# jscant/PointVS

Hardware: AMD Instinct MI355X
Metric: protein-ligand graphs/sec fwd+bwd (+Adam step), 3-layer EGNN ch=32, ~2k nodes r=10A (higher is better)
Workload: dtype f32

## Files before the change

### pointvs_amd/csrc/graph_prepare.hip

```cpp
#include "common.h"
#include "profile.h"
#include <hipcub/hipcub.hpp>

namespace {

__global__ void k_extract(const int64_t* __restrict__ ei, const int64_t* __restrict__ ea, int A,
                          int N, int E, int32_t* row32, int32_t* col32, int32_t* ids,
                          uint8_t* etype_in, int32_t* status) {
    int e = blockIdx.x * blockDim.x + threadIdx.x;
    if (e >= E) return;
    int64_t r = ei[e], c = ei[(size_t)E + e];
    int bad = 0;
    if (r < 0 || r >= N || c < 0 || c >= N) { bad |= 1; r = 0; c = 0; }
    row32[e] = (int32_t)r;
    col32[e] = (int32_t)c;
    ids[e] = e;
    if (A > 0) {
        int hot = -1, ones = 0, other = 0;
        for (int a = 0; a < A; ++a) {
            int64_t v = ea[(size_t)e * A + a];
            if (v == 1) { ones++; hot = a; }
            else if (v != 0) other = 1;
        }
        if (ones != 1 || other) { bad |= 2; if (hot < 0) hot = 0; }
// ... 208 lines not shown
    int p = blockIdx.x * blockDim.x + threadIdx.x;
    if (p < E) iota[p] = p;
}

__global__ void k_init_split(int n_graphs, const int32_t* __restrict__ edge_ptr, int32_t* __restrict__ split,
                             int32_t* __restrict__ status) {
    const int g = blockIdx.x * blockDim.x + threadIdx.x;
    if (g == 0) *status = 0;
    if (g < n_graphs) split[g] = edge_ptr[g + 1];
}

__global__ void k_run_starts(const int64_t* __restrict__ rows, int N, int E, int n_graphs,
                             const int32_t* __restrict__ status, const int32_t* __restrict__ node_ptr,
                             const int32_t* __restrict__ edge_ptr, const int32_t* __restrict__ split,
                             int2* __restrict__ rec, int32_t* __restrict__ unsafe,
                             int32_t* __restrict__ rowptr, float* __restrict__ inv_deg) {
    const int n = blockIdx.x * blockDim.x + threadIdx.x;
    if (n >= N) return;
    if (n == N - 1) rowptr[N] = E;
    const bool broken = (*status & 5) != 0;
    if (n == 0) *unsafe = broken;
    if (broken) {
        rec[n] = make_int2(0, 0);
        rowptr[n] = n == 0 ? 0 : E;
        inv_deg[n] = 1.0f;
        return;
    }
    int lo = 0, hi = n_graphs;
    while (hi - lo > 1) {
        const int mid = (lo + hi) >> 1;
        if (node_ptr[mid] <= n) lo = mid; else hi = mid;
    }
    const int g = lo;
    const int a0 = edge_ptr[g], a1 = split[g], b1 = edge_ptr[g + 1];
    int f0 = a0, l0 = a1, f1 = a0, l1 = a1, f2 = a1, l2 = b1, f3 = a1, l3 = b1;
    while (f0 < l0 || f1 < l1 || f2 < l2 || f3 < l3) {
        const int m0 = (f0 + l0) >> 1, m1 = (f1 + l1) >> 1, m2 = (f2 + l2) >> 1, m3 = (f3 + l3) >> 1;
        const int64_t v0 = f0 < l0 ? rows[m0] : 0, v1 = f1 < l1 ? rows[m1] : 0;
        const int64_t v2 = f2 < l2 ? rows[m2] : 0, v3 = f3 < l3 ? rows[m3] : 0;
        if (f0 < l0) { if (v0 < n) f0 = m0 + 1; else l0 = m0; }
        if (f1 < l1) { if (v1 < n + 1) f1 = m1 + 1; else l1 = m1; }
        if (f2 < l2) { if (v2 < n) f2 = m2 + 1; else l2 = m2; }
        if (f3 < l3) { if (v3 < n + 1) f3 = m3 + 1; else l3 = m3; }
    }
    const int sa = f0, sa_next = f1, sb = f2, sb_next = f3;
    const int d = (sa_next - sa) + (sb_next - sb);
    const int first = a0 + (sa - a0) + (sb - a1);
    rowptr[n] = first;
    rec[n] = make_int2(first - sa, first + (sa_next - sa) - sb);
    inv_deg[n] = 1.0f / (float)(d > 1 ? d : 1);
}

__device__ __forceinline__ int prep_code(long long v) { return v == 0 ? 0 : v == 1 ? 1 : 2; }

template <bool VEC, int AMAX>
__global__ void __launch_bounds__(kPrepThreads)
k_place_stream(const int64_t* __restrict__ ei, const int64_t* __restrict__ ea, int A, int N, int E, int n_graphs,
               const int32_t* __restrict__ node_ptr, const int32_t* __restrict__ edge_ptr,
               const int32_t* __restrict__ split, const int2* __restrict__ rec, const int32_t* __restrict__ unsafe,
               int32_t* __restrict__ row, int32_t* __restrict__ col, uint8_t* __restrict__ etype,
               int32_t* __restrict__ perm, int32_t* __restrict__ status) {
    __shared__ unsigned short codes[kPrepWaves][kPlaceEdges / 2][64 * AMAX];
    const int lane = threadIdx.x & 63, wv = threadIdx.x >> 6;
    const long long cb = ((long long)blockIdx.x * kPrepWaves + wv) * (64 * kPlaceEdges);
    PrepSeg s;
    s.g = graph_of_edge(edge_ptr, n_graphs, (int)min(cb + lane, (long long)E - 1), E, kPlaceEdges);
    if (cb >= E) return;
    const int64_t* cols = ei + (size_t)E;
    long long r[kPlaceEdges], c[kPlaceEdges];
#pragma unroll
    for (int j = 0; j < kPlaceEdges; ++j) {
        const long long e = cb + 64 * j + lane;
        r[j] = e < E ? (long long)prep_load_once(ei + e) : 0;
        c[j] = e < E ? (long long)prep_load_once(cols + e) : 0;
    }
    const bool by_pieces = A > 0 && A <= AMAX;
    if (by_pieces) {
        const size_t words = (size_t)E * A;
        pvs_ll2 av[kPlaceEdges / 2][AMAX];
#pragma unroll
        for (int jj = 0; jj < kPlaceEdges / 2; ++jj)
#pragma unroll
            for (int q = 0; q < AMAX; ++q) {
                av[jj][q] = pvs_ll2{0, 0};
                if (q >= A) continue;
                const size_t w0 = (size_t)(cb + 128 * jj) * A + 2 * (size_t)(q * 64 + lane);
                if (VEC && w0 + 1 < words) {
                    av[jj][q] = prep_load_once(reinterpret_cast<const pvs_ll2*>(ea + w0));
                } else {
                    if (w0 < words) av[jj][q].x = ea[w0];
                    if (w0 + 1 < words) av[jj][q].y = ea[w0 + 1];
                }
            }
#pragma unroll
        for (int jj = 0; jj < kPlaceEdges / 2; ++jj)
#pragma unroll
            for (int q = 0; q < AMAX; ++q)
                if (q < A) codes[wv][jj][q * 64 + lane] = (unsigned short)(prep_code(av[jj][q].x) | prep_code(av[jj][q].y) << 8);
        __builtin_amdgcn_fence(__ATOMIC_RELEASE, "wavefront");
        __builtin_amdgcn_wave_barrier();
        __builtin_amdgcn_fence(__ATOMIC_ACQUIRE, "wavefront");
    }
    const bool safe_graph = *unsafe != 0;
    prep_seg_load(s, node_ptr, edge_ptr);
    int second_from = split[s.g];
    int bad = 0;
#pragma unroll
    for (int j = 0; j < kPlaceEdges; ++j) {
        const long long el = cb + 64 * j + lane;
        if (el >= E) continue;
        const int e = (int)el;
        if (prep_seg_advance(s, e, n_graphs, node_ptr, edge_ptr)) second_from = split[s.g];
        long long cc = c[j];
        bool col_bad = false;
        if (cc < 0 || cc >= N) { bad |= 1; cc = 0; col_bad = true; }
        if (cc < s.n_lo || cc >= s.n_hi) { bad |= 4; col_bad = true; }
        int hot = -1;
        if (A > 0) {
            int ones = 0, other = 0;
            if (by_pieces) {
                const unsigned char* mine = reinterpret_cast<const unsigned char*>(codes[wv][j >> 1]) + ((j & 1) * 64 + lane) * A;
                for (int a = 0; a < A; ++a) {
                    const int k = mine[a];
                    if (k == 1) { ones++; hot = a; } else if (k != 0) other = 1;
                }
            } else {
                for (int a = 0; a < A; ++a) {
                    const int64_t v = ea[(size_t)e * A + a];
                    if (v == 1) { ones++; hot = a; } else if (v != 0) other = 1;
                }
            }
            if (ones != 1 || other) { bad |= 2; if (hot < 0) hot = 0; }
        }
        if (safe_graph) {
            row[e] = 0; col[e] = 0; perm[e] = e;
            if (etype) etype[e] = 0;
            continue;
        }
        const int rr = (int)r[j];
        const int2 t = rec[rr];
        const int pos = e + (e >= second_from ? t.y : t.x);
        row[pos] = rr;
        col[pos] = col_bad ? rr : (int)cc;
        if (etype) etype[pos] = (uint8_t)hot;
        perm[pos] = e;
    }
    if (bad) atomicOr(status, bad);
}

constexpr int kCscMaxCols = 4096;
constexpr int kCscWaves = 4;
constexpr int kCscTargetChunks = 2048;
constexpr int kCscAhead = 8;

struct CscChunk { int begin, end, node_lo, width, g; };

__device__ __forceinline__ CscChunk csc_chunk(int wid, int cpg, int stride, int n_graphs, int N, int E,
                                              const int32_t* __restrict__ node_ptr,
                                              const int32_t* __restrict__ edge_ptr) {
    CscChunk c;
    c.g = wid / cpg;
    const int k = wid - c.g * cpg;
    if (c.g >= n_graphs) { c.begin = c.end = 0; c.node_lo = 0; c.width = 0; return c; }
    const int e0 = min(max(edge_ptr[c.g], 0), E), e1 = min(max(edge_ptr[c.g + 1], e0), E);
    const int len = (((e1 - e0) + cpg - 1) / cpg + 63) & ~63;
    c.begin = min(e0 + k * len, e1);
    c.end = min(c.begin + len, e1);
    c.node_lo = min(max(node_ptr[c.g], 0), N);
    c.width = min(max(node_ptr[c.g + 1], c.node_lo), N) - c.node_lo;
    return c;
}

template <class T, class Sink>
__device__ __forceinline__ void csc_walk_chunk(const int32_t* __restrict__ col, const CscChunk& c, int lane, T* tab,
                                               unsigned char* tag, Sink&& sink) {
    for (int q0 = c.begin; q0 < c.end; q0 += 64 * kCscAhead) {
        int keys[kCscAhead];
#pragma unroll
        for (int u = 0; u < kCscAhead; ++u)
            keys[u] = col[min(q0 + 64 * u + lane, c.end - 1)];
#pragma unroll
        for (int u = 0; u < kCscAhead; ++u) {
            const int k = min(max(keys[u] - c.node_lo, 0), c.width - 1);
            keys[u] = q0 + 64 * u + lane < c.end ? k : -1;
        }
#pragma unroll
        for (int u = 0; u < kCscAhead; ++u) {
            const int p = q0 + 64 * u + lane;
            const int key = keys[u];
            const bool live = key >= 0;
            if (q0 + 64 * u >= c.end) break;
            int leader = lane, rank = 0, members = 1;
            if (live) tag[key] = (unsigned char)lane;
            __builtin_amdgcn_fence(__ATOMIC_RELEASE, "wavefront");
            __builtin_amdgcn_wave_barrier();
            __builtin_amdgcn_fence(__ATOMIC_ACQUIRE, "wavefront");
            const bool lost = live && tag[key] != (unsigned char)lane;
            unsigned long long pending = __ballot(lost);
            while (pending) {
                const int l0 = __builtin_ctzll(pending);
                const int k0 = __builtin_amdgcn_readlane(key, l0);
                const unsigned long long grp = __ballot(live && key == k0);
                if (live && key == k0) {
                    leader = __builtin_ctzll(grp);
                    rank = __popcll(grp & ((1ull << lane) - 1ull));
                    members = __popcll(grp);
                }
                pending &= ~grp;
            }
            int slot = 0;
            if (live && rank == 0) {
                slot = (int)tab[key];
                tab[key] = (T)(slot + members);
            }
            slot = __shfl(slot, leader, 64) + rank;
            if (live) sink(slot, p);
            __builtin_amdgcn_fence(__ATOMIC_RELEASE, "wavefront");
            __builtin_amdgcn_wave_barrier();
            __builtin_amdgcn_fence(__ATOMIC_ACQUIRE, "wavefront");
        }
    }
}

template <bool PLACE>
__global__ void __launch_bounds__(64 * kCscWaves)
k_csc_pass(const int32_t* __restrict__ col, int n_graphs, int N, int E, const int32_t* __restrict__ node_ptr,
           const int32_t* __restrict__ edge_ptr, int cpg, int stride, int32_t* __restrict__ cnt,
           int32_t* __restrict__ cedge, int32_t* __restrict__ status) {
    extern __shared__ int32_t csc_lds[];
    const int lane = threadIdx.x & 63, wv = threadIdx.x >> 6;
    const int bpg = cpg / kCscWaves;
    const int xcd = blockIdx.x & 7, j = blockIdx.x >> 3;
    const int g_of_block = (j / bpg) * 8 + xcd;
    const int wid = g_of_block * cpg + (j % bpg) * kCscWaves + wv;
    CscChunk c = csc_chunk(g_of_block < n_graphs ? wid : n_graphs * cpg, cpg, stride, n_graphs, N, E, node_ptr, edge_ptr);
    if (c.width > stride) {
        if (lane == 0) atomicOr(status, 4);
        c.width = stride;
    }
    if (c.width <= 0) return;
    if (PLACE && (*status & 4)) {
        for (int p = c.begin + lane; p < c.end; p += 64) cedge[p] = p;
        return;
    }
    int32_t* tab = csc_lds + wv * (stride + stride / 4);
    unsigned char* tag = reinterpret_cast<unsigned char*>(tab + stride);
    int32_t* mine = cnt + (size_t)wid * stride;
    for (int i = lane; i < c.width; i += 64) tab[i] = PLACE ? mine[i] : 0;
    __builtin_amdgcn_fence(__ATOMIC_RELEASE, "wavefront");
    __builtin_amdgcn_wave_barrier();
    __builtin_amdgcn_fence(__ATOMIC_ACQUIRE, "wavefront");
    if (PLACE) {
        csc_walk_chunk(col, c, lane, tab, tag, [&](int slot, int p) { cedge[min(max(slot, 0), E - 1)] = p; });
        return;
    }
    for (int q0 = c.begin; q0 < c.end; q0 += 64 * kCscAhead) {
        int keys[kCscAhead];
#pragma unroll
        for (int u = 0; u < kCscAhead; ++u)
            keys[u] = col[min(q0 + 64 * u + lane, c.end - 1)];
#pragma unroll
        for (int u = 0; u < kCscAhead; ++u) {
            if (q0 + 64 * u >= c.end) break;
            const int k = min(max(keys[u] - c.node_lo, 0), c.width - 1);
            if (q0 + 64 * u + lane < c.end) atomicAdd(&tab[k], 1);
        }
    }
    if (!PLACE) {
        __builtin_amdgcn_fence(__ATOMIC_RELEASE, "wavefront");
        __builtin_amdgcn_wave_barrier();
        __builtin_amdgcn_fence(__ATOMIC_ACQUIRE, "wavefront");
        for (int i = lane; i < c.width; i += 64) mine[i] = tab[i];
    }
}

template <int NW>
__global__ void __launch_bounds__(64 * NW)
k_csc_place_tiles(const int32_t* __restrict__ col, int n_graphs, int N, int E, const int32_t* __restrict__ node_ptr,
                  const int32_t* __restrict__ edge_ptr, int cpg, int stride, const int32_t* __restrict__ cnt,
                  const int32_t* __restrict__ colptr, int32_t* __restrict__ cedge, int32_t* __restrict__ status, int cap) {
    extern __shared__ int32_t csc_lds[];
    const int lane = threadIdx.x & 63, wv = threadIdx.x >> 6, tid = threadIdx.x;
    const int tpg = cpg / NW;
    const int g = blockIdx.x / tpg, tl = blockIdx.x - g * tpg;
    if (g >= n_graphs) return;
    const int k0 = g * cpg + tl * NW;
    CscChunk c = csc_chunk(k0 + wv, cpg, stride, n_graphs, N, E, node_ptr, edge_ptr);
    if (c.width > stride) {
        if (lane == 0) atomicOr(status, 4);
        c.width = stride;
    }
    if (c.width <= 0) return;
    if (*status & 4) {
        for (int p = c.begin + lane; p < c.end; p += 64) cedge[p] = p;
        return;
    }
    const CscChunk first = csc_chunk(k0, cpg, stride, n_graphs, N, E, node_ptr, edge_ptr);
    const CscChunk last = csc_chunk(k0 + NW - 1, cpg, stride, n_graphs, N, E, node_ptr, edge_ptr);
    const int tile_begin = first.begin, tile_len = last.end - first.begin;
    const int width = c.width;
    if (tile_len > cap || tile_len > 65535) {
        int32_t* tab = csc_lds + wv * (stride + stride / 4);
        unsigned char* tag = reinterpret_cast<unsigned char*>(tab + stride);
        const int32_t* mine = cnt + (size_t)(k0 + wv) * stride;
        for (int i = lane; i < width; i += 64) tab[i] = mine[i];
        __builtin_amdgcn_fence(__ATOMIC_RELEASE, "wavefront");
        __builtin_amdgcn_wave_barrier();
        __builtin_amdgcn_fence(__ATOMIC_ACQUIRE, "wavefront");
        csc_walk_chunk(col, c, lane, tab, tag, [&](int slot, int p) { cedge[min(max(slot, 0), E - 1)] = p; });
        return;
    }
    int32_t* lstart = csc_lds;
    int32_t* gbase = lstart + stride + 64;
    unsigned short* tabs = reinterpret_cast<unsigned short*>(gbase + stride);
    unsigned char* tags = reinterpret_cast<unsigned char*>(tabs + NW * stride);
    unsigned short* list = reinterpret_cast<unsigned short*>(tags + NW * stride);
    const bool last_tile = tl == tpg - 1;
    for (int i = tid; i < width; i += 64 * NW) {
        const int32_t* src = cnt + (size_t)k0 * stride + i;
        const int s0 = src[0];
        const int s_end = last_tile ? colptr[c.node_lo + i + 1] : src[(size_t)NW * stride];
        gbase[i] = s0;
        lstart[i] = s_end - s0;
#pragma unroll
        for (int k = 0; k < NW; ++k) tabs[k * stride + i] = (unsigned short)(src[(size_t)k * stride] - s0);
    }
    __syncthreads();
    {
        __shared__ int32_t wave_tot[NW];
        const int per = (width + 64 * NW - 1) / (64 * NW), a = tid * per;
        int sum = 0;
        for (int i = a; i < min(a + per, width); ++i) sum += lstart[i];
        int inc = sum;
#pragma unroll
        for (int o = 1; o < 64; o <<= 1) {
            const int up = __shfl_up(inc, o, 64);
            if (lane >= o) inc += up;
        }
        if (lane == 63) wave_tot[wv] = inc;
        __syncthreads();
        int run = inc - sum;
        for (int k = 0; k < wv; ++k) run += wave_tot[k];
        for (int i = a; i < min(a + per, width); ++i) {
            const int v = lstart[i];
            lstart[i] = run;
            run += v;
        }
        if (tid == 64 * NW - 1) lstart[width] = run;
    }
    __syncthreads();
    for (int i = tid; i < width; i += 64 * NW) {
        const int base = lstart[i];
#pragma unroll
        for (int k = 0; k < NW; ++k) tabs[k * stride + i] = (unsigned short)(tabs[k * stride + i] + base);
    }
    __syncthreads();
    csc_walk_chunk(col, c, lane, tabs + wv * stride, tags + wv * stride,
                   [&](int slot, int p) { list[min(max(slot, 0), cap - 1)] = (unsigned short)(p - tile_begin); });
    __syncthreads();
    const int hw = tid >> 5, l32 = tid & 31;
    for (int cc = hw; cc < width; cc += 2 * NW) {
        const int a = lstart[cc], b = lstart[cc + 1], dst = gbase[cc];
        for (int i = a + l32; i < b; i += 32)
            cedge[min(max(dst + i - a, 0), E - 1)] = tile_begin + (int)list[min(i, cap - 1)];
    }
}

__device__ __forceinline__ int csc_graph_of_node(const int32_t* __restrict__ node_ptr, int n_graphs, int n) {
    int lo = 0, hi = n_graphs;
    while (hi - lo > 1) {
        const int mid = (lo + hi) >> 1;
        if (node_ptr[mid] <= n) lo = mid; else hi = mid;
    }
    return lo;
}

int csc_chunks_per_graph(int n_graphs) {
    int cpg = kCscTargetChunks / (n_graphs > 0 ? n_graphs : 1);
    cpg = (cpg / kCscWaves) * kCscWaves;
    if (cpg < kCscWaves) cpg = kCscWaves;
    if (cpg > 128) cpg = 128;
    return cpg;
}
int csc_blocks(int n_graphs, int cpg) { return ((n_graphs + 7) / 8) * (cpg / kCscWaves) * 8; }
int csc_stride(int max_graph_nodes) { return (max_graph_nodes + 63) & ~63; }
bool csc_counting_ok(int max_graph_nodes) { return max_graph_nodes > 0 && max_graph_nodes <= kCscMaxCols; }

struct RunsWs {
    int32_t *iota, *keys_tmp, *split, *unsafe, *csc_cnt, *indeg;
    int2* rec;
    void* sort_tmp;
    size_t sort_bytes;
};

size_t carve_runs(PvsArena& a, int N, int E, int B, int max_graph_nodes, RunsWs* w) {
    const size_t e = (size_t)(E > 0 ? E : 1);
    RunsWs t;
    t.split = a.take<int32_t>((size_t)B + 1);
    t.unsafe = a.take<int32_t>(1);
    t.rec = a.take<int2>((size_t)N);
    t.csc_cnt = nullptr;
    t.indeg = nullptr;
    t.iota = t.keys_tmp = nullptr;
    t.sort_tmp = nullptr;
    t.sort_bytes = 0;
    if (csc_counting_ok(max_graph_nodes)) {
        t.csc_cnt = a.take<int32_t>((size_t)B * csc_chunks_per_graph(B) * csc_stride(max_graph_nodes));
        t.indeg = a.take<int32_t>((size_t)N + 1);
    }
    t.iota = a.take<int32_t>(e);
    t.keys_tmp = a.take<int32_t>(e);
    t.sort_bytes = sort_temp_bytes(E > 0 ? E : 1, key_bits(N > 1 ? N : 2));
    t.sort_tmp = a.take<char>(t.sort_bytes);
    if (w) *w = t;
    return a.off;
}

__global__ void k_csc_totals(const int32_t* __restrict__ cnt, int N, int n_graphs, const int32_t* __restrict__ node_ptr,
                             int cpg, int stride, int32_t* __restrict__ indeg, const int32_t* __restrict__ status) {
    const int n = blockIdx.x * blockDim.x + threadIdx.x;
    if (n >= N) return;
    if (*status & 4) { indeg[n] = 0; return; }
    const int g = csc_graph_of_node(node_ptr, n_graphs, n);
    const int c = n - node_ptr[g];
    int t0 = 0, t1 = 0, t2 = 0, t3 = 0;
    if (c >= 0 && c < stride) {
        const int32_t* src = cnt + (size_t)g * cpg * stride + c;
        for (int k = 0; k < cpg; k += 4) {
            t0 += src[(size_t)k * stride];
            t1 += src[(size_t)(k + 1) * stride];
            t2 += src[(size_t)(k + 2) * stride];
            t3 += src[(size_t)(k + 3) * stride];
        }
    }
    indeg[n] = (t0 + t1) + (t2 + t3);
}

__global__ void __launch_bounds__(256) k_csc_colptr(int32_t* __restrict__ cnt, const int32_t* __restrict__ indeg, int N, int E,
                                                    int n_graphs, const int32_t* __restrict__ node_ptr,
                                                    const int32_t* __restrict__ edge_ptr, int cpg, int stride,
                                                    int32_t* __restrict__ colptr, const int32_t* __restrict__ status) {
    __shared__ int32_t wave_tot[4], front_tot[4];
    const int t = threadIdx.x, lane = t & 63, wv = t >> 6;
    if (*status & 4) {
        for (int i = (blockIdx.y * gridDim.x + blockIdx.x) * 256 + t; i <= N; i += gridDim.x * gridDim.y * 256) colptr[i] = 0;
        return;
    }
    for (int g = blockIdx.y; g < n_graphs; g += gridDim.y) {
        if (g == n_graphs - 1 && blockIdx.x == 0 && t == 0) colptr[N] = E;
        const int n0 = node_ptr[g], width = min(node_ptr[g + 1] - n0, stride);
        const int c0 = blockIdx.x * 256;
        if (c0 >= width) continue;
        int front = 0;
        for (int c = t; c < c0; c += 256) front += indeg[n0 + c];
        const int c = c0 + t;
        const int mine = c < width ? indeg[n0 + c] : 0;
        int inc = mine;
#pragma unroll
        for (int o = 1; o < 64; o <<= 1) {
            const int up = __shfl_up(inc, o, 64);
            if (lane >= o) inc += up;
            front += __shfl_xor(front, o, 64);
        }
        if (lane == 63) wave_tot[wv] = inc;
        if (lane == 0) front_tot[wv] = front;
        __syncthreads();
        int run = edge_ptr[g] + (front_tot[0] + front_tot[1]) + (front_tot[2] + front_tot[3]) + inc - mine;
        for (int k = 0; k < wv; ++k) run += wave_tot[k];
        if (c < width) {
            colptr[n0 + c] = run;
            int32_t* slot = cnt + (size_t)g * cpg * stride + c;
            for (int k = 0; k < cpg; k += 4) {
                const int v0 = slot[(size_t)k * stride], v1 = slot[(size_t)(k + 1) * stride];
                const int v2 = slot[(size_t)(k + 2) * stride], v3 = slot[(size_t)(k + 3) * stride];
                slot[(size_t)k * stride] = run;
                slot[(size_t)(k + 1) * stride] = run + v0;
                slot[(size_t)(k + 2) * stride] = run + v0 + v1;
                slot[(size_t)(k + 3) * stride] = run + v0 + v1 + v2;
                run += (v0 + v1) + (v2 + v3);
            }
        }
        __syncthreads();
    }
}

}

extern "C" size_t pvs_graph_prepare_runs_workspace_bytes(int32_t n_nodes, int32_t n_edges, int32_t n_graphs,
                                                         int32_t max_graph_nodes) {
    PvsArena a(nullptr, 0);
    return carve_runs(a, n_nodes, n_edges, n_graphs, max_graph_nodes, nullptr) + 256;
}

extern "C" int pvs_graph_prepare_runs(const int64_t* edge_index, const int64_t* edge_attr, int32_t n_edge_attr,
                                      int32_t N, int32_t E, int32_t n_graphs, const int32_t* node_ptr,
                                      const int32_t* edge_ptr, int32_t* rowptr, int32_t* row, int32_t* col,
                                      uint8_t* etype, int32_t* perm, int32_t* colptr, int32_t* cedge, float* inv_deg,
                                      int32_t* status, int32_t max_graph_nodes, void* workspace,
                                      size_t workspace_bytes, pvs_stream_t stream_) {
    hipStream_t stream = (hipStream_t)stream_;
    PVS_REQUIRE(N > 0 && E >= 0 && n_graphs > 0, "pvs_graph_prepare_runs: bad sizes N=%d E=%d B=%d", N, E, n_graphs);
    PVS_REQUIRE(max_graph_nodes >= 0, "pvs_graph_prepare_runs: bad max_graph_nodes %d", max_graph_nodes);
    PVS_REQUIRE(n_edge_attr >= 0 && n_edge_attr <= 255, "pvs_graph_prepare_runs: bad n_edge_attr %d", n_edge_attr);
    PVS_REQUIRE(n_edge_attr == 0 || (edge_attr && etype), "pvs_graph_prepare_runs: edge_attr/etype NULL");
    PVS_REQUIRE(node_ptr && edge_ptr, "pvs_graph_prepare_runs: node_ptr / edge_ptr NULL");
    PVS_REQUIRE((colptr == nullptr) == (cedge == nullptr), "pvs_graph_prepare_runs: colptr and cedge go together");
    PvsArena arena(workspace, workspace_bytes);
    RunsWs w;
    carve_runs(arena, N, E, n_graphs, max_graph_nodes, &w);
    PVS_REQUIRE(arena.ok(), "pvs_graph_prepare_runs: workspace too small (%zu < %zu)", workspace_bytes, arena.off);
    PvsProfScope prof(stream, PVS_PROF_PREPARE);
    const int T = 256;
    k_init_split<<<(n_graphs + T - 1) / T > 0 ? (n_graphs + T - 1) / T : 1, T, 0, stream>>>(n_graphs, edge_ptr, w.split, status);
    PVS_CHECK_LAUNCH();
    if (E > 0) {
        const int scan_edges = kPrepThreads * kScanEdges;
        k_scan_rows<<<(E + scan_edges - 1) / scan_edges, kPrepThreads, 0, stream>>>(edge_index, N, E, n_graphs, node_ptr,
                                                                                           edge_ptr, w.split, status);
        PVS_CHECK_LAUNCH();
    }
    k_run_starts<<<(N + T - 1) / T, T, 0, stream>>>(edge_index, N, E, n_graphs, status, node_ptr, edge_ptr, w.split, w.rec,
                                                    w.unsafe, rowptr, inv_deg);
    PVS_CHECK_LAUNCH();
    if (E > 0) {
        const bool vec = ((uintptr_t)edge_attr & 15) == 0;
        const int place_edges = kPrepThreads * kPlaceEdges;
        const int blocks = (E + place_edges - 1) / place_edges;
        auto place = n_edge_attr <= 3 ? (vec ? k_place_stream<true, 3> : k_place_stream<false, 3>)
                                      : (vec ? k_place_stream<true, 8> : k_place_stream<false, 8>);
        place<<<blocks, kPrepThreads, 0, stream>>>(edge_index, edge_attr, n_edge_attr, N, E, n_graphs, node_ptr, edge_ptr,
                                                   w.split, w.rec, w.unsafe, row, col, n_edge_attr ? etype : nullptr, perm,
                                                   status);
        PVS_CHECK_LAUNCH();
    }
    if (!cedge) return 0;
    static const bool force_sort = [] { const char* e = getenv("PVS_CSC_SORT"); return e && e[0] == '1'; }();
    if (w.csc_cnt && !force_sort) {
        const int cpg = csc_chunks_per_graph(n_graphs), stride = csc_stride(max_graph_nodes);
        const int waves = n_graphs * cpg, blocks = csc_blocks(n_graphs, cpg);
        const size_t lds = (size_t)kCscWaves * (stride + stride / 4) * sizeof(int32_t);
        if (lds > 48 * 1024) {
            PVS_CHECK_HIP(hipFuncSetAttribute((const void*)k_csc_pass<false>, hipFuncAttributeMaxDynamicSharedMemorySize, (int)lds));
            PVS_CHECK_HIP(hipFuncSetAttribute((const void*)k_csc_pass<true>, hipFuncAttributeMaxDynamicSharedMemorySize, (int)lds));
        }
        if (E > 0) {
            k_csc_pass<false><<<blocks, 64 * kCscWaves, lds, stream>>>(col, n_graphs, N, E, node_ptr, edge_ptr, cpg, stride,
                                                                        w.csc_cnt, nullptr, status);
            PVS_CHECK_LAUNCH();
        } else {
            PVS_CHECK_HIP(hipMemsetAsync(w.csc_cnt, 0, (size_t)waves * stride * sizeof(int32_t), stream));
        }
        k_csc_totals<<<(N + T - 1) / T, T, 0, stream>>>(w.csc_cnt, N, n_graphs, node_ptr, cpg, stride, w.indeg, status);
        PVS_CHECK_LAUNCH();
        k_csc_colptr<<<dim3((max_graph_nodes + 255) / 256, n_graphs < 65535 ? n_graphs : 65535), 256, 0, stream>>>(w.csc_cnt, w.indeg, N, E, n_graphs, node_ptr,
                                                                                         edge_ptr, cpg, stride, colptr, status);
        PVS_CHECK_LAUNCH();
        if (E > 0) {
            const char* tiles_env = getenv("PVS_CSC_TILES");
            const bool tiles_on = !(tiles_env && tiles_env[0] == '0');
            const int budget = 160 * 1024 - 256;
            auto fixed_bytes = [&](int nw) { return (size_t)(stride + 64) * 4 + (size_t)stride * 4 + (size_t)nw * stride * 3; };
            int nw = (cpg % 8 == 0 && fixed_bytes(8) + 2 * 32768 <= (size_t)budget) ? 8 : 4;
            int cap = ((int)budget - (int)fixed_bytes(nw)) / 2;
            if (cap > 65535) cap = 65535;
            const bool forced = tiles_env && tiles_env[0] == '2';
            const double avg_run = (double)E / ((double)(N > 0 ? N : 1) * (double)(cpg / nw));
            if (tiles_on && (avg_run >= 10.0 || forced) && cap >= 8192 && (size_t)nw * (stride + stride / 4) * 4 <= (size_t)budget) {
                const int tiles = n_graphs * (cpg / nw);
                if (nw == 8) {
                    PVS_CHECK_HIP(hipFuncSetAttribute((const void*)k_csc_place_tiles<8>, hipFuncAttributeMaxDynamicSharedMemorySize, budget));
                    k_csc_place_tiles<8><<<tiles, 64 * 8, budget, stream>>>(col, n_graphs, N, E, node_ptr, edge_ptr, cpg, stride,
                                                                           w.csc_cnt, colptr, cedge, status, cap);
                } else {
                    PVS_CHECK_HIP(hipFuncSetAttribute((const void*)k_csc_place_tiles<4>, hipFuncAttributeMaxDynamicSharedMemorySize, budget));
                    k_csc_place_tiles<4><<<tiles, 64 * 4, budget, stream>>>(col, n_graphs, N, E, node_ptr, edge_ptr, cpg, stride,
                                                                           w.csc_cnt, colptr, cedge, status, cap);
                }
            } else {
                k_csc_pass<true><<<blocks, 64 * kCscWaves, lds, stream>>>(col, n_graphs, N, E, node_ptr, edge_ptr, cpg, stride,
                                                                           w.csc_cnt, cedge, status);
            }
            PVS_CHECK_LAUNCH();
        }
        return 0;
    }
    if (E > 0) {
        size_t tb = w.sort_bytes;
        const int bits = key_bits(N > 1 ? N : 2);
        k_iota<<<(E + 255) / 256, 256, 0, stream>>>(E, w.iota);
        PVS_CHECK_LAUNCH();
        PVS_CHECK_HIP(hipcub::DeviceRadixSort::SortPairs(w.sort_tmp, tb, col, w.keys_tmp, w.iota, cedge, E, 0,
                                                         bits, stream));
    }
    k_lower_bounds<<<(N + 1 + T - 1) / T, T, 0, stream>>>(w.keys_tmp, E, N, colptr, nullptr);
    PVS_CHECK_LAUNCH();
    return 0;
}

namespace {
}

size_t pvs_build_csc_workspace_bytes(int N, int E) {
    const size_t e = (size_t)(E > 0 ? E : 1);
    return 2 * pvs_align_up(e * sizeof(int32_t), 256) +
           pvs_align_up(sort_temp_bytes((int)e, key_bits(N > 1 ? N : 2)), 256) + 512;
}

int pvs_build_csc(hipStream_t stream, const int32_t* col, int E, int N, int32_t* colptr, int32_t* cedge,
                  void* workspace, size_t workspace_bytes) {
    PVS_REQUIRE(workspace_bytes >= pvs_build_csc_workspace_bytes(N, E) - 512, "build_csc: workspace too small");
    PvsArena a(workspace, workspace_bytes);
    const size_t e = (size_t)(E > 0 ? E : 1);
    int32_t* iota = a.take<int32_t>(e);
    int32_t* keys = a.take<int32_t>(e);
    const int bits = key_bits(N > 1 ? N : 2);
    size_t tb = sort_temp_bytes((int)e, bits);
    void* tmp = a.take<char>(tb);
    if (E > 0) {
        k_iota<<<(E + 255) / 256, 256, 0, stream>>>(E, iota);
        PVS_CHECK_LAUNCH();
        PVS_CHECK_HIP(hipcub::DeviceRadixSort::SortPairs(tmp, tb, col, keys, iota, cedge, E, 0, bits, stream));
    }
    k_lower_bounds<<<(N + 1 + 255) / 256, 256, 0, stream>>>(keys, E, N, colptr, nullptr);
    PVS_CHECK_LAUNCH();
    return 0;
}

namespace {
template <bool FILL>
__global__ void __launch_bounds__(256)
k_filter_ligand(PvsGraph g, const uint8_t* __restrict__ bp, int capacity, int32_t* __restrict__ cnt,
                const int32_t* __restrict__ rowptr_out, int32_t* __restrict__ row_out,
                int32_t* __restrict__ col_out, uint8_t* __restrict__ etype_out, int32_t* __restrict__ status) {
    const int lane = threadIdx.x & 63;
    const int i = (blockIdx.x * 256 + threadIdx.x) >> 6;
    if (i >= g.n_nodes) return;
    const bool lig_row = bp[i] == 0;
    const int p0 = g.rowptr[i], p1 = g.rowptr[i + 1];
    int done = 0;
    const int base = FILL ? rowptr_out[i] : 0;
    if (FILL && rowptr_out[g.n_nodes] > capacity) {
        if (i == 0 && lane == 0) atomicOr(status, 4);
        return;
    }
    for (int pb = p0; pb < p1; pb += 64) {
        const int p = pb + lane;
        int c = 0;
        bool keep = false;
        if (p < p1) {
            c = g.col[p];
            keep = lig_row || bp[c] == 0;
        }
        const unsigned long long m = __ballot(keep);
        if (FILL && keep) {
            const int q = base + done + __popcll(m & ((1ull << lane) - 1ull));
            row_out[q] = i;
            col_out[q] = c;
            if (etype_out) etype_out[q] = g.etype[p];
        }
        done += __popcll(m);
    }
    if (!FILL && lane == 0) cnt[i] = done;
}
}

extern "C" size_t pvs_graph_filter_workspace_bytes(int32_t N) {
    size_t sb = 0;
    (void)hipcub::DeviceScan::ExclusiveSum(nullptr, sb, (const int32_t*)nullptr, (int32_t*)nullptr, N + 1);
    return pvs_align_up(((size_t)N + 1) * sizeof(int32_t), 256) + pvs_align_up(sb, 256) + 512;
}

extern "C" int pvs_graph_filter_ligand_edges(const PvsGraph* full, const uint8_t* bp, int32_t capacity,
                                             int32_t* rowptr_out, int32_t* row_out, int32_t* col_out,
                                             uint8_t* etype_out, int32_t* status, void* workspace,
                                             size_t workspace_bytes, pvs_stream_t stream_) {
    hipStream_t s = (hipStream_t)stream_;
    PVS_REQUIRE(full && bp && rowptr_out && row_out && col_out && status && full->rowptr && full->col,
                "pvs_graph_filter_ligand_edges: NULL");
    PVS_REQUIRE(!full->n_edges_dev, "pvs_graph_filter_ligand_edges: needs a graph with a host-side edge count");
    PVS_REQUIRE(etype_out == nullptr || full->etype, "pvs_graph_filter_ligand_edges: graph has no edge classes");
    const int N = full->n_nodes;
    PVS_REQUIRE(workspace_bytes >= pvs_graph_filter_workspace_bytes(N) - 512, "filter workspace too small");
    PvsArena a(workspace, workspace_bytes);
    int32_t* cnt = a.take<int32_t>((size_t)N + 1);
    size_t sb = 0;
    (void)hipcub::DeviceScan::ExclusiveSum(nullptr, sb, (const int32_t*)nullptr, (int32_t*)nullptr, N + 1);
    void* tmp = a.take<char>(sb);
    PVS_CHECK_HIP(hipMemsetAsync(status, 0, sizeof(int32_t), s));
    PVS_CHECK_HIP(hipMemsetAsync(cnt + N, 0, sizeof(int32_t), s));
    const int blocks = (N + 3) / 4;
    k_filter_ligand<false><<<blocks, 256, 0, s>>>(*full, bp, capacity, cnt, nullptr, nullptr, nullptr, nullptr, status);
    PVS_CHECK_LAUNCH();
    PVS_CHECK_HIP(hipcub::DeviceScan::ExclusiveSum(tmp, sb, cnt, rowptr_out, N + 1, s));
    k_filter_ligand<true><<<blocks, 256, 0, s>>>(*full, bp, capacity, nullptr, rowptr_out, row_out, col_out,
                                                 etype_out, status);
    PVS_CHECK_LAUNCH();
    return 0;
}

namespace {
template <bool TO_INPUT>
__global__ void k_permute_rows(const float* __restrict__ src, float* __restrict__ dst,
                               const int32_t* __restrict__ perm, int E, int width) {
    long long total = (long long)E * width;
    for (long long i = (long long)blockIdx.x * blockDim.x + threadIdx.x; i < total;
         i += (long long)gridDim.x * blockDim.x) {
        int e = (int)(i / width), c = (int)(i % width);
        int o = perm[e];
        if (TO_INPUT) dst[(size_t)o * width + c] = src[i];
        else dst[i] = src[(size_t)o * width + c];
    }
}
}

extern "C" int pvs_rows_to_input_order(const float* src, float* dst, const int32_t* perm,
                                       int32_t E, int32_t width, pvs_stream_t stream) {
    if (E <= 0) return 0;
    long long total = (long long)E * width;
    int blocks = (int)((total + 255) / 256 < 8192 ? (total + 255) / 256 : 8192);
    k_permute_rows<true><<<blocks, 256, 0, (hipStream_t)stream>>>(src, dst, perm, E, width);
    PVS_CHECK_LAUNCH();
    return 0;
}

extern "C" int pvs_rows_to_sorted_order(const float* src, float* dst, const int32_t* perm,
                                        int32_t E, int32_t width, pvs_stream_t stream) {
    if (E <= 0) return 0;
    long long total = (long long)E * width;
    int blocks = (int)((total + 255) / 256 < 8192 ? (total + 255) / 256 : 8192);
    k_permute_rows<false><<<blocks, 256, 0, (hipStream_t)stream>>>(src, dst, perm, E, width);
    PVS_CHECK_LAUNCH();
    return 0;
}

// ... 96 lines not shown
```

Measured before the change: 5901.

## Fuse CSC count/total/colptr stages into two-kernel tiled count and place path

The tiled CSC build now uses its own per-tile count kernel and folds the per-node totals, column-pointer scan and local slot computation into the place kernel. This replaces the old four-kernel sequence (per-wave count, totals, colptr, place). The walk also prefetches the next batch of column keys and skips the tag-and-ballot grouping when a DPP neighbour compare shows no duplicate keys, with a bitwise match path when many lanes collide. The output scatter is unrolled across several columns. In exchange, each place block redundantly sums all tile rows for its graph, and the LDS layout and guard conditions become more complex.

```diff
diff --git a/pointvs_amd/csrc/graph_prepare.hip b/pointvs_amd/csrc/graph_prepare.hip
--- a/pointvs_amd/csrc/graph_prepare.hip
+++ b/pointvs_amd/csrc/graph_prepare.hip
@@ -384,6 +384,8 @@
 constexpr int kCscWaves = 4;
 constexpr int kCscTargetChunks = 2048;
 constexpr int kCscAhead = 8;
+constexpr int kCscMatchFrom = 2;
+constexpr int kCscOut = 4;
 
 struct CscChunk { int begin, end, node_lo, width, g; };
 
@@ -406,15 +408,21 @@
 template <class T, class Sink>
 __device__ __forceinline__ void csc_walk_chunk(const int32_t* __restrict__ col, const CscChunk& c, int lane, T* tab,
                                                unsigned char* tag, Sink&& sink) {
+    int ahead[kCscAhead];
+#pragma unroll
+    for (int u = 0; u < kCscAhead; ++u)
+        ahead[u] = col[min(c.begin + 64 * u + lane, max(c.end, 1) - 1)];
     for (int q0 = c.begin; q0 < c.end; q0 += 64 * kCscAhead) {
         int keys[kCscAhead];
 #pragma unroll
-        for (int u = 0; u < kCscAhead; ++u)
-            keys[u] = col[min(q0 + 64 * u + lane, c.end - 1)];
-#pragma unroll
         for (int u = 0; u < kCscAhead; ++u) {
-            const int k = min(max(keys[u] - c.node_lo, 0), c.width - 1);
+            const int k = min(max(ahead[u] - c.node_lo, 0), c.width - 1);
             keys[u] = q0 + 64 * u + lane < c.end ? k : -1;
+        }
+        if (q0 + 64 * kCscAhead < c.end) {
+#pragma unroll
+            for (int u = 0; u < kCscAhead; ++u)
+                ahead[u] = col[min(q0 + 64 * (kCscAhead + u) + lane, c.end - 1)];
         }
 #pragma unroll
         for (int u = 0; u < kCscAhead; ++u) {
@@ -423,33 +431,70 @@
             const bool live = key >= 0;
             if (q0 + 64 * u >= c.end) break;
             int leader = lane, rank = 0, members = 1;
-            if (live) tag[key] = (unsigned char)lane;
-            __builtin_amdgcn_fence(__ATOMIC_RELEASE, "wavefront");
-            __builtin_amdgcn_wave_barrier();
-            __builtin_amdgcn_fence(__ATOMIC_ACQUIRE, "wavefront");
-            const bool lost = live && tag[key] != (unsigned char)lane;
-            unsigned long long pending = __ballot(lost);
-            while (pending) {
-                const int l0 = __builtin_ctzll(pending);
-                const int k0 = __builtin_amdgcn_readlane(key, l0);
-                const unsigned long long grp = __ballot(live && key == k0);
-                if (live && key == k0) {
+            bool grouped = false;
+            const int below = __builtin_amdgcn_update_dpp(-2, key, 0x138 , 0xf, 0xf, false);
+            const bool shared = __ballot(live && key <= below) != 0ull;
+            if (shared) {
+                if (live) tag[key] = (unsigned char)lane;
+                __builtin_amdgcn_fence(__ATOMIC_RELEASE, "wavefront");
+                __builtin_amdgcn_wave_barrier();
+                __builtin_amdgcn_fence(__ATOMIC_ACQUIRE, "wavefront");
+                const int winner = live ? (int)tag[key] : lane;
+                unsigned long long pending = __ballot(winner != lane);
+                grouped = pending != 0ull;
+                if (__popcll(pending) > kCscMatchFrom) {
+                    uint32_t lo = ~0u, hi = ~0u;
+#pragma unroll
+                    for (int b = 0; b < 6; ++b) {
+                        const uint32_t ones = 0u - ((uint32_t)(winner >> b) & 1u);
+                        const unsigned long long with_bit = __ballot(ones != 0u);
+                        lo &= ~((uint32_t)with_bit ^ ones);
+                        hi &= ~((uint32_t)(with_bit >> 32) ^ ones);
+                    }
+                    const unsigned long long grp = ((unsigned long long)hi << 32) | lo;
                     leader = __builtin_ctzll(grp);
                     rank = __popcll(grp & ((1ull << lane) - 1ull));
                     members = __popcll(grp);
+                    pending = 0ull;
                 }
-                pending &= ~grp;
+                while (pending) {
+                    const int l0 = __builtin_ctzll(pending);
+                    const int k0 = __builtin_amdgcn_readlane(key, l0);
+                    const unsigned long long grp = __ballot(live && key == k0);
+                    if (live && key == k0) {
+                        leader = __builtin_ctzll(grp);
+                        rank = __popcll(grp & ((1ull << lane) - 1ull));
+                        members = __popcll(grp);
+                    }
+                    pending &= ~grp;
+                }
             }
             int slot = 0;
             if (live && rank == 0) {
                 slot = (int)tab[key];
                 tab[key] = (T)(slot + members);
             }
-            slot = __shfl(slot, leader, 64) + rank;
+            if (grouped) slot = __shfl(slot, leader, 64) + rank;
             if (live) sink(slot, p);
             __builtin_amdgcn_fence(__ATOMIC_RELEASE, "wavefront");
             __builtin_amdgcn_wave_barrier();
             __builtin_amdgcn_fence(__ATOMIC_ACQUIRE, "wavefront");
+        }
+    }
+}
+
+template <class Add>
+__device__ __forceinline__ void csc_count_chunk(const int32_t* __restrict__ col, const CscChunk& c, int lane, Add&& add) {
+    for (int q0 = c.begin; q0 < c.end; q0 += 64 * kCscAhead) {
+        int keys[kCscAhead];
+#pragma unroll
+        for (int u = 0; u < kCscAhead; ++u)
+            keys[u] = col[min(q0 + 64 * u + lane, c.end - 1)];
+#pragma unroll
+        for (int u = 0; u < kCscAhead; ++u) {
+            if (q0 + 64 * u >= c.end) break;
+            const int k = min(max(keys[u] - c.node_lo, 0), c.width - 1);
+            if (q0 + 64 * u + lane < c.end) add(k);
         }
     }
 }
@@ -506,16 +551,82 @@
     }
 }
 
+
 template <int NW>
 __global__ void __launch_bounds__(64 * NW)
-k_csc_place_tiles(const int32_t* __restrict__ col, int n_graphs, int N, int E, const int32_t* __restrict__ node_ptr,
-                  const int32_t* __restrict__ edge_ptr, int cpg, int stride, const int32_t* __restrict__ cnt,
-                  const int32_t* __restrict__ colptr, int32_t* __restrict__ cedge, int32_t* __restrict__ status, int cap) {
+k_csc_count_tiles(const int32_t* __restrict__ col, int n_graphs, int N, int E, const int32_t* __restrict__ node_ptr,
+                  const int32_t* __restrict__ edge_ptr, int cpg, int stride, int32_t* __restrict__ tcnt,
+                  int32_t* __restrict__ status) {
     extern __shared__ int32_t csc_lds[];
     const int lane = threadIdx.x & 63, wv = threadIdx.x >> 6, tid = threadIdx.x;
     const int tpg = cpg / NW;
     const int g = blockIdx.x / tpg, tl = blockIdx.x - g * tpg;
     if (g >= n_graphs) return;
+    CscChunk c = csc_chunk(g * cpg + tl * NW + wv, cpg, stride, n_graphs, N, E, node_ptr, edge_ptr);
+    if (c.width > stride) {
+        if (lane == 0) atomicOr(status, 4);
+        c.width = stride;
+    }
+    if (c.width <= 0) return;
+    for (int i = tid; i < c.width; i += 64 * NW) csc_lds[i] = 0;
+    __syncthreads();
+    csc_count_chunk(col, c, lane, [&](int k) { atomicAdd(&csc_lds[k], 1); });
+    __syncthreads();
+    int32_t* mine = tcnt + (size_t)blockIdx.x * stride;
+    for (int i = tid; i < c.width; i += 64 * NW) mine[i] = csc_lds[i];
+}
+
+template <int NW>
+__device__ __forceinline__ void csc_tile_scan(int32_t* a, int32_t* b, int width, int tid, int32_t* wave_tot) {
+    const int lane = tid & 63, wv = tid >> 6;
+    const int per = (width + 64 * NW - 1) / (64 * NW), lo = tid * per, hi = min(lo + per, width);
+    int sa = 0, sb = 0;
+    for (int i = lo; i < hi; ++i) {
+        sa += a[i];
+        if (b) sb += b[i];
+    }
+    int ia = sa, ib = sb;
+#pragma unroll
+    for (int o = 1; o < 64; o <<= 1) {
+        const int ua = __shfl_up(ia, o, 64), ub = __shfl_up(ib, o, 64);
+        if (lane >= o) { ia += ua; ib += ub; }
+    }
+    if (lane == 63) { wave_tot[wv] = ia; wave_tot[NW + wv] = ib; }
+    __syncthreads();
+    int ra = ia - sa, rb = ib - sb;
+    for (int k = 0; k < wv; ++k) { ra += wave_tot[k]; rb += wave_tot[NW + k]; }
+    for (int i = lo; i < hi; ++i) {
+        const int va = a[i];
+        a[i] = ra;
+        ra += va;
+        if (b) {
+            const int vb = b[i];
+            b[i] = rb;
+            rb += vb;
+        }
+    }
+    if (tid == 64 * NW - 1) {
+        a[width] = ra;
+        if (b) b[width] = rb;
+    }
+    __syncthreads();
+}
+
+template <int NW>
+__global__ void __launch_bounds__(64 * NW)
+k_csc_place_tiles(const int32_t* __restrict__ col, int n_graphs, int N, int E, const int32_t* __restrict__ node_ptr,
+                  const int32_t* __restrict__ edge_ptr, int cpg, int stride, const int32_t* __restrict__ tcnt,
+                  int32_t* __restrict__ colptr, int32_t* __restrict__ cedge, int32_t* __restrict__ status, int cap) {
+    extern __shared__ int32_t csc_lds[];
+    __shared__ int32_t wave_tot[2 * NW];
+    const int lane = threadIdx.x & 63, wv = threadIdx.x >> 6, tid = threadIdx.x;
+    const int tpg = cpg / NW;
+    const int g = blockIdx.x / tpg, tl = blockIdx.x - g * tpg;
+    const bool broken = (*status & 4) != 0;
+    if (broken)
+        for (int i = blockIdx.x * 64 * NW + tid; i <= N; i += gridDim.x * 64 * NW) colptr[i] = 0;
+    if (g >= n_graphs) return;
+    if (!broken && g == n_graphs - 1 && tl == 0 && tid == 0) colptr[N] = E;
     const int k0 = g * cpg + tl * NW;
     CscChunk c = csc_chunk(k0 + wv, cpg, stride, n_graphs, N, E, node_ptr, edge_ptr);
     if (c.width > stride) {
@@ -523,7 +634,7 @@
         c.width = stride;
     }
     if (c.width <= 0) return;
-    if (*status & 4) {
+    if (broken) {
         for (int p = c.begin + lane; p < c.end; p += 64) cedge[p] = p;
         return;
     }
@@ -531,70 +642,104 @@
     const CscChunk last = csc_chunk(k0 + NW - 1, cpg, stride, n_graphs, N, E, node_ptr, edge_ptr);
     const int tile_begin = first.begin, tile_len = last.end - first.begin;
     const int width = c.width;
-    if (tile_len > cap || tile_len > 65535) {
-        int32_t* tab = csc_lds + wv * (stride + stride / 4);
-        unsigned char* tag = reinterpret_cast<unsigned char*>(tab + stride);
-        const int32_t* mine = cnt + (size_t)(k0 + wv) * stride;
-        for (int i = lane; i < width; i += 64) tab[i] = mine[i];
-        __builtin_amdgcn_fence(__ATOMIC_RELEASE, "wavefront");
-        __builtin_amdgcn_wave_barrier();
-        __builtin_amdgcn_fence(__ATOMIC_ACQUIRE, "wavefront");
-        csc_walk_chunk(col, c, lane, tab, tag, [&](int slot, int p) { cedge[min(max(slot, 0), E - 1)] = p; });
-        return;
-    }
+    const int e0 = min(max(edge_ptr[g], 0), E);
+    const int32_t* rows = tcnt + (size_t)g * tpg * stride;
+    const bool direct = tile_len > cap || tile_len > 65535;
     int32_t* lstart = csc_lds;
     int32_t* gbase = lstart + stride + 64;
     unsigned short* tabs = reinterpret_cast<unsigned short*>(gbase + stride);
     unsigned char* tags = reinterpret_cast<unsigned char*>(tabs + NW * stride);
     unsigned short* list = reinterpret_cast<unsigned short*>(tags + NW * stride);
-    const bool last_tile = tl == tpg - 1;
+    int32_t* slots = gbase + stride;
+    unsigned char* tags_direct = reinterpret_cast<unsigned char*>(slots + NW * stride);
+    int32_t* tot = direct ? lstart : reinterpret_cast<int32_t*>(list);
+
+    uint32_t* words = reinterpret_cast<uint32_t*>(slots);
+    for (int i = tid; i < (direct ? NW * stride : NW * stride / 2); i += 64 * NW) words[i] = 0u;
+    __syncthreads();
+
+    if (direct) {
+        csc_count_chunk(col, c, lane, [&](int k) { atomicAdd(&slots[wv * stride + k], 1); });
+    } else {
+        uint32_t* mine = words + wv * (stride / 2);
+        csc_count_chunk(col, c, lane, [&](int k) { atomicAdd(&mine[k >> 1], 1u << ((k & 1) * 16)); });
+    }
+
     for (int i = tid; i < width; i += 64 * NW) {
-        const int32_t* src = cnt + (size_t)k0 * stride + i;
-        const int s0 = src[0];
-        const int s_end = last_tile ? colptr[c.node_lo + i + 1] : src[(size_t)NW * stride];
-        gbase[i] = s0;
-        lstart[i] = s_end - s0;
-#pragma unroll
-        for (int k = 0; k < NW; ++k) tabs[k * stride + i] = (unsigned short)(src[(size_t)k * stride] - s0);
+        int total = 0, front = 0;
+#pragma unroll 4
+        for (int t = 0; t < tpg; ++t) {
+            const int v = rows[(size_t)t * stride + i];
+            total += v;
+            front += t < tl ? v : 0;
+        }
+        tot[i] = total;
+        gbase[i] = front;
     }
     __syncthreads();
-    {
-        __shared__ int32_t wave_tot[NW];
-        const int per = (width + 64 * NW - 1) / (64 * NW), a = tid * per;
-        int sum = 0;
-        for (int i = a; i < min(a + per, width); ++i) sum += lstart[i];
-        int inc = sum;
-#pragma unroll
-        for (int o = 1; o < 64; o <<= 1) {
-            const int up = __shfl_up(inc, o, 64);
-            if (lane >= o) inc += up;
-        }
-        if (lane == 63) wave_tot[wv] = inc;
+
+    if (direct) {
+        csc_tile_scan<NW>(tot, nullptr, width, tid, wave_tot);
+        for (int i = tid; i < width; i += 64 * NW) {
+            int run = e0 + tot[i];
+            if (tl == 0) colptr[c.node_lo + i] = run;
+            run += gbase[i];
+#pragma unroll
+            for (int k = 0; k < NW; ++k) {
+                const int v = slots[k * stride + i];
+                slots[k * stride + i] = run;
+                run += v;
+            }
+        }
         __syncthreads();
-        int run = inc - sum;
-        for (int k = 0; k < wv; ++k) run += wave_tot[k];
-        for (int i = a; i < min(a + per, width); ++i) {
-            const int v = lstart[i];
-            lstart[i] = run;
+        csc_walk_chunk(col, c, lane, slots + wv * stride, tags_direct + wv * stride,
+                       [&](int slot, int p) { cedge[min(max(slot, 0), E - 1)] = p; });
+        return;
+    }
+    for (int i = tid; i < width; i += 64 * NW) {
+        int run = 0;
+#pragma unroll
+        for (int k = 0; k < NW; ++k) {
+            const int v = tabs[k * stride + i];
+            tabs[k * stride + i] = (unsigned short)run;
             run += v;
         }
-        if (tid == 64 * NW - 1) lstart[width] = run;
+        lstart[i] = run;
     }
     __syncthreads();
+    csc_tile_scan<NW>(lstart, tot, width, tid, wave_tot);
     for (int i = tid; i < width; i += 64 * NW) {
-        const int base = lstart[i];
+        const int base = lstart[i], first_of_column = e0 + tot[i];
 #pragma unroll
         for (int k = 0; k < NW; ++k) tabs[k * stride + i] = (unsigned short)(tabs[k * stride + i] + base);
+        if (tl == 0) colptr[c.node_lo + i] = first_of_column;
+        gbase[i] += first_of_column;
     }
     __syncthreads();
+
     csc_walk_chunk(col, c, lane, tabs + wv * stride, tags + wv * stride,
                    [&](int slot, int p) { list[min(max(slot, 0), cap - 1)] = (unsigned short)(p - tile_begin); });
     __syncthreads();
+
     const int hw = tid >> 5, l32 = tid & 31;
-    for (int cc = hw; cc < width; cc += 2 * NW) {
-        const int a = lstart[cc], b = lstart[cc + 1], dst = gbase[cc];
-        for (int i = a + l32; i < b; i += 32)
-            cedge[min(max(dst + i - a, 0), E - 1)] = tile_begin + (int)list[min(i, cap - 1)];
+    for (int cc = hw; cc < width; cc += 2 * NW * kCscOut) {
+        int a[kCscOut], b[kCscOut], dst[kCscOut], v[kCscOut];
+#pragma unroll
+        for (int u = 0; u < kCscOut; ++u) {
+            const int cu = min(cc + 2 * NW * u, width - 1);
+            a[u] = lstart[cu];
+            b[u] = cc + 2 * NW * u < width ? lstart[cu + 1] : a[u];
+            dst[u] = gbase[cu];
+        }
+#pragma unroll
+        for (int u = 0; u < kCscOut; ++u) v[u] = (int)list[min(a[u] + l32, cap - 1)];
+#pragma unroll
+        for (int u = 0; u < kCscOut; ++u)
+            if (a[u] + l32 < b[u]) cedge[min(max(dst[u] + l32, 0), E - 1)] = tile_begin + v[u];
+#pragma unroll
+        for (int u = 0; u < kCscOut; ++u)
+            for (int i = a[u] + 32 + l32; i < b[u]; i += 32)
+                cedge[min(max(dst[u] + i - a[u], 0), E - 1)] = tile_begin + (int)list[min(i, cap - 1)];
     }
 }
 
@@ -770,23 +915,6 @@
     if (w.csc_cnt && !force_sort) {
         const int cpg = csc_chunks_per_graph(n_graphs), stride = csc_stride(max_graph_nodes);
         const int waves = n_graphs * cpg, blocks = csc_blocks(n_graphs, cpg);
-        const size_t lds = (size_t)kCscWaves * (stride + stride / 4) * sizeof(int32_t);
-        if (lds > 48 * 1024) {
-            PVS_CHECK_HIP(hipFuncSetAttribute((const void*)k_csc_pass<false>, hipFuncAttributeMaxDynamicSharedMemorySize, (int)lds));
-            PVS_CHECK_HIP(hipFuncSetAttribute((const void*)k_csc_pass<true>, hipFuncAttributeMaxDynamicSharedMemorySize, (int)lds));
-        }
-        if (E > 0) {
-            k_csc_pass<false><<<blocks, 64 * kCscWaves, lds, stream>>>(col, n_graphs, N, E, node_ptr, edge_ptr, cpg, stride,
-                                                                        w.csc_cnt, nullptr, status);
-            PVS_CHECK_LAUNCH();
-        } else {
-            PVS_CHECK_HIP(hipMemsetAsync(w.csc_cnt, 0, (size_t)waves * stride * sizeof(int32_t), stream));
-        }
-        k_csc_totals<<<(N + T - 1) / T, T, 0, stream>>>(w.csc_cnt, N, n_graphs, node_ptr, cpg, stride, w.indeg, status);
-        PVS_CHECK_LAUNCH();
-        k_csc_colptr<<<dim3((max_graph_nodes + 255) / 256, n_graphs < 65535 ? n_graphs : 65535), 256, 0, stream>>>(w.csc_cnt, w.indeg, N, E, n_graphs, node_ptr,
-                                                                                         edge_ptr, cpg, stride, colptr, status);
-        PVS_CHECK_LAUNCH();
         if (E > 0) {
             const char* tiles_env = getenv("PVS_CSC_TILES");
             const bool tiles_on = !(tiles_env && tiles_env[0] == '0');
@@ -797,21 +925,42 @@
             if (cap > 65535) cap = 65535;
             const bool forced = tiles_env && tiles_env[0] == '2';
             const double avg_run = (double)E / ((double)(N > 0 ? N : 1) * (double)(cpg / nw));
-            if (tiles_on && (avg_run >= 10.0 || forced) && cap >= 8192 && (size_t)nw * (stride + stride / 4) * 4 <= (size_t)budget) {
+            if (tiles_on && (avg_run >= 10.0 || forced) && cap >= 8192 && cap >= 2 * stride + 2 &&
+                (size_t)(2 * stride + 64) * 4 + (size_t)nw * stride * 5 <= (size_t)budget) {
                 const int tiles = n_graphs * (cpg / nw);
-                if (nw == 8) {
-                    PVS_CHECK_HIP(hipFuncSetAttribute((const void*)k_csc_place_tiles<8>, hipFuncAttributeMaxDynamicSharedMemorySize, budget));
-                    k_csc_place_tiles<8><<<tiles, 64 * 8, budget, stream>>>(col, n_graphs, N, E, node_ptr, edge_ptr, cpg, stride,
-                                                                           w.csc_cnt, colptr, cedge, status, cap);
-                } else {
-                    PVS_CHECK_HIP(hipFuncSetAttribute((const void*)k_csc_place_tiles<4>, hipFuncAttributeMaxDynamicSharedMemorySize, budget));
-                    k_csc_place_tiles<4><<<tiles, 64 * 4, budget, stream>>>(col, n_graphs, N, E, node_ptr, edge_ptr, cpg, stride,
-                                                                           w.csc_cnt, colptr, cedge, status, cap);
-                }
-            } else {
-                k_csc_pass<true><<<blocks, 64 * kCscWaves, lds, stream>>>(col, n_graphs, N, E, node_ptr, edge_ptr, cpg, stride,
-                                                                           w.csc_cnt, cedge, status);
+                int32_t* tcnt = w.csc_cnt;
+                auto count = nw == 8 ? k_csc_count_tiles<8> : k_csc_count_tiles<4>;
+                auto place = nw == 8 ? k_csc_place_tiles<8> : k_csc_place_tiles<4>;
+                PVS_CHECK_HIP(hipFuncSetAttribute((const void*)place, hipFuncAttributeMaxDynamicSharedMemorySize, budget));
+                count<<<tiles, 64 * nw, (size_t)stride * sizeof(int32_t), stream>>>(col, n_graphs, N, E, node_ptr, edge_ptr, cpg,
+                                                                                   stride, tcnt, status);
+                PVS_CHECK_LAUNCH();
+                place<<<tiles, 64 * nw, budget, stream>>>(col, n_graphs, N, E, node_ptr, edge_ptr, cpg, stride, tcnt, colptr,
+                                                          cedge, status, cap);
+                PVS_CHECK_LAUNCH();
+                return 0;
             }
+        }
+        const size_t lds = (size_t)kCscWaves * (stride + stride / 4) * sizeof(int32_t);
+        if (lds > 48 * 1024) {
+            PVS_CHECK_HIP(hipFuncSetAttribute((const void*)k_csc_pass<false>, hipFuncAttributeMaxDynamicSharedMemorySize, (int)lds));
+            PVS_CHECK_HIP(hipFuncSetAttribute((const void*)k_csc_pass<true>, hipFuncAttributeMaxDynamicSharedMemorySize, (int)lds));
+        }
+        if (E > 0) {
+            k_csc_pass<false><<<blocks, 64 * kCscWaves, lds, stream>>>(col, n_graphs, N, E, node_ptr, edge_ptr, cpg, stride,
+                                                                        w.csc_cnt, nullptr, status);
+            PVS_CHECK_LAUNCH();
+        } else {
+            PVS_CHECK_HIP(hipMemsetAsync(w.csc_cnt, 0, (size_t)waves * stride * sizeof(int32_t), stream));
+        }
+        k_csc_totals<<<(N + T - 1) / T, T, 0, stream>>>(w.csc_cnt, N, n_graphs, node_ptr, cpg, stride, w.indeg, status);
+        PVS_CHECK_LAUNCH();
+        k_csc_colptr<<<dim3((max_graph_nodes + 255) / 256, n_graphs < 65535 ? n_graphs : 65535), 256, 0, stream>>>(w.csc_cnt, w.indeg, N, E, n_graphs, node_ptr,
+                                                                                         edge_ptr, cpg, stride, colptr, status);
+        PVS_CHECK_LAUNCH();
+        if (E > 0) {
+            k_csc_pass<true><<<blocks, 64 * kCscWaves, lds, stream>>>(col, n_graphs, N, E, node_ptr, edge_ptr, cpg, stride,
+                                                                       w.csc_cnt, cedge, status);
             PVS_CHECK_LAUNCH();
         }
         return 0;
```

Measured after the change: 5954 (median of 6 runs). No clear change (+0.9%).
